# llsurreal919/Reduce-Complexity-for-intra-coding-of-VVC

Hardware: NVIDIA B200
Metric: all-intra 1080p10 CTUs/sec (exhaustive RMD sweep: intra pred + SAD/SATD + mode cost + candidate lists) (higher is better)
Workload: dtype int16 samples / int32 arithmetic / f64 costs

## Files before the change

### vvc_intra_b200/csrc/vvcb_core.cuh

```cuda
#pragma once
#include <stdint.h>
#include "../../include/vvc_intra_b200.h"

#if defined(__CUDACC__)
#define VHD __host__ __device__ __forceinline__
#else
#define VHD inline
#endif

namespace vvcb {

constexpr int kLineMax   = 140;
constexpr int kNumSets   = 4;
constexpr int kSlotLineWords = 54 * 32;
constexpr int kNumClasses = 6;
constexpr int kNumKinds   = 3;
constexpr int kNumBuckets = kNumClasses * kNumKinds;
#ifndef VVCB_ITEM_TASKS
#define VVCB_ITEM_TASKS 512
#endif
constexpr int kItemTasks = VVCB_ITEM_TASKS;

VHD int vmin(int a, int b) { return a < b ? a : b; }
VHD int vmax(int a, int b) { return a > b ? a : b; }
VHD int vabs(int a) { return a < 0 ? -a : a; }
VHD int vlog2(int v)
{
#if defined(__CUDA_ARCH__)
  return 31 - __clz(v);
#else
  return 31 - __builtin_clz((unsigned)v);
#endif
}
VHD int vsad(int a, int b, int c)
{
#if defined(__CUDA_ARCH__)
  return (int)__sad(a, b, (unsigned)c);
#else
  return c + (a < b ? b - a : a - b);
#endif
}

VHD uint32_t pack_u16x2(int lo, int hi) { return (uint32_t)lo | ((uint32_t)hi << 16); }
VHD uint32_t max_u16x2(uint32_t a, uint32_t b)
{
#if defined(__CUDA_ARCH__)
  return __vmaxu2(a, b);
#else
  const uint32_t al = a & 0xffffu, bl = b & 0xffffu, ah = a >> 16, bh = b >> 16;
  return (al > bl ? al : bl) | ((ah > bh ? ah : bh) << 16);
#endif
}
VHD int add_halves_u16x2(uint32_t w, int acc)
{
#if defined(__CUDA_ARCH__)
  return (int)__dp2a_lo(w, 0x00000101u, (unsigned)acc);
#else
  return acc + (int)(w & 0xffffu) + (int)(w >> 16);
#endif
}

struct ModeParam {
  int16_t  angle;
  uint16_t inv_angle;
  uint8_t  is_ver;
  uint8_t  ref_filter;
  uint8_t  interp;
  uint8_t  pdpc;
  int8_t   ang_scale;
  uint8_t  pad[3];
};

VHD int wide_angle(int w, int h, int mode)
{
  const int shiftTab[6] = { 0, 6, 10, 12, 14, 15 };
  if (mode > 1 && mode <= 66) {
    const int d = vabs(vlog2(w) - vlog2(h));
    if (w > h && mode < 2 + shiftTab[d]) mode += 65;
    else if (h > w && mode > 66 - shiftTab[d]) mode -= 65;
  }
  return mode;
}

VHD ModeParam make_mode_param(int w, int h, int mode, int mrl)
{
  const int angTab[32] = { 0, 1, 2, 3, 4, 6, 8, 10, 12, 14, 16, 18, 20, 23, 26, 29,
                           32, 35, 39, 45, 51, 57, 64, 73, 86, 102, 128, 171, 256, 341, 512, 1024 };
  const int invTab[32] = { 0, 16384, 8192, 5461, 4096, 2731, 2048, 1638, 1365, 1170, 1024, 910, 819, 712, 630, 565,
                           512, 468, 420, 364, 321, 287, 256, 224, 191, 161, 128, 96, 64, 48, 32, 16 };
  const int filtThr[8] = { 24, 24, 24, 14, 2, 0, 0, 0 };
  ModeParam p = {};
  const int predMode = wide_angle(w, h, mode);
  p.is_ver = predMode >= 34;
  p.pdpc   = mrl == 0;
  int absAng = 0;
  const int angMode = p.is_ver ? predMode - 50 : -(predMode - 18);
  if (mode > 1) {
    const int a = vabs(angMode);
    absAng      = angTab[a];
    p.inv_angle = (uint16_t)invTab[a];
    p.angle     = (int16_t)(angMode < 0 ? -absAng : absAng);
    if (angMode < 0) p.pdpc = 0;
    else if (angMode > 0) {
      const int side = p.is_ver ? h : w;
      const int sc   = vmin(2, vlog2(side) - (vlog2(3 * p.inv_angle - 2) - 8));
      p.ang_scale = (int8_t)sc;
      p.pdpc = p.pdpc && sc >= 0;
    }
  }
  if (mrl || mode == 1) return p;
  if (mode == 0) { p.ref_filter = w * h > 32; return p; }
// ... 53 lines not shown
  s.unitsX = w / s.S; s.unitsY = h / s.S;
  s.lanes = (s.tile == 1 || s.tile == 2) ? (w * h) / 32 : s.unitsX * s.unitsY;
  s.lgLanes  = vlog2(s.lanes);
  s.lgTilesX = s.S == 8 ? lw - 3 : (s.tile == 1 ? lw - 3 : lw - 2);
  return s;
}

struct WorkItem {
  uint32_t visit;
  uint16_t slot_begin;
  uint16_t slot_count;
};

struct LineGeom {
  int w, h, mrl, n;
  int lo[5], hi[5];
  int first;
};
constexpr int kNoInterval = 0x3fffffff;

VHD LineGeom make_line_geom(const vvcb_rmd_visit& v, int w, int h, int mrl)
{
  LineGeom g;
  g.w = w; g.h = h; g.mrl = mrl;
  const int C = 2 * h + 2 * mrl + 1;
  g.n = C + 2 * w;
  g.lo[0] = v.n_below_left  ? h - 4 * v.n_below_left : kNoInterval;  g.hi[0] = h;
  g.lo[1] = v.n_left        ? 2 * h - 4 * v.n_left   : kNoInterval;  g.hi[1] = 2 * h;
  g.lo[2] = v.avail_al      ? 2 * h                  : kNoInterval;  g.hi[2] = C;
  g.lo[3] = v.n_above       ? C                      : kNoInterval;  g.hi[3] = C + 4 * v.n_above;
  g.lo[4] = v.n_above_right ? C + w                  : kNoInterval;  g.hi[4] = C + w + 4 * v.n_above_right;
  g.first = -1;
#pragma unroll
  for (int k = 4; k >= 0; k--) if (g.lo[k] != kNoInterval) g.first = g.lo[k];
  return g;
}

VHD int line_source(const LineGeom& g, int i)
{
  int src = g.first;
#pragma unroll
  for (int k = 0; k < 5; k++)
    if (i >= g.lo[k]) src = i < g.hi[k] ? i : g.hi[k] - 1;
  return src;
}

VHD void line_pos(const LineGeom& g, int i, bool& isLeft, int& k, int& dx, int& dy)
{
  const int nLeft = 2 * g.h + g.mrl;
  if (i < nLeft) { isLeft = true;  k = nLeft - i;  dx = -1 - g.mrl; dy = -1 - g.mrl + k; }
  else           { isLeft = false; k = i - nLeft;  dx = -1 - g.mrl + k; dy = -1 - g.mrl; }
}

struct Rom {
  uint32_t filt[2][32];
  ModeParam mode[6][6][VVCB_NUM_LUMA_MODE];
  uint8_t angOrder[6][6][65];
  uint8_t mip4[18 * 16 * 4], mip8[10 * 16 * 8], mip16[6 * 64 * 7];
  uint8_t mipOff4[18], mipSh4[18], mipOff8[10], mipSh8[10], mipOff16[6], mipSh16[6];
};

template <int R, int C> VHD void wht_rows_rc(int (&d)[R][C])
{
#pragma unroll
  for (int y = 0; y < R; y++)
#pragma unroll
    for (int len = 1; len < C; len <<= 1)
#pragma unroll
      for (int i = 0; i < C; i += 2 * len)
#pragma unroll
        for (int x = i; x < i + len; x++) {
          const int a = d[y][x], b = d[y][x + len];
          d[y][x] = a + b; d[y][x + len] = a - b;
        }
}
template <int N> VHD void wht_rows(int (&d)[N][N]) { wht_rows_rc<N, N>(d); }

template <int R, int C> VHD void wht_cols_rc(int (&d)[R][C])
{
#pragma unroll
  for (int x = 0; x < C; x++)
#pragma unroll
    for (int len = 1; len < R; len <<= 1)
#pragma unroll
      for (int i = 0; i < R; i += 2 * len)
#pragma unroll
        for (int y = i; y < i + len; y++) {
          const int a = d[y][x], b = d[y + len][x];
          d[y][x] = a + b; d[y + len][x] = a - b;
        }
}

template <int N> VHD int wht_cols_abs_sum(int (&d)[N][N])
{
#pragma unroll
  for (int x = 0; x < N; x++)
#pragma unroll
    for (int len = 1; len < N / 2; len <<= 1)
#pragma unroll
      for (int i = 0; i < N; i += 2 * len)
#pragma unroll
        for (int y = i; y < i + len; y++) {
          const int a = d[y][x], b = d[y + len][x];
          d[y][x] = a + b; d[y + len][x] = a - b;
        }
  int s = 0;
#pragma unroll
  for (int x = 0; x < N; x++)
#pragma unroll
    for (int y = 0; y < N / 2; y++) s += vmax(vabs(d[y][x]), vabs(d[y + N / 2][x]));
  return 2 * s;
}
// ... 62 lines not shown
        }
      }
    } else {
      const int scale = p.ang_scale;
      const int lim = vmin(3 << scale, mw);
#pragma unroll
      for (int j = 0; j < C; j++) {
        const int c = c0 + j;
        if (c < lim) {
          const int wL  = 32 >> ((2 * c) >> scale);
          const int off = (256 + (c + 1) * (int)p.inv_angle) >> 9;
#pragma unroll
          for (int i = 0; i < R; i++) {
            const int l = side[r0 + i + off + 1];
            q[i][j] = q[i][j] + ((wL * (l - q[i][j]) + 32) >> 6);
          }
        }
      }
    }
  }
}

template <int R, int C> VHD void pred_planar_dc_unit(const int16_t* top, const int16_t* left, int kind, bool pdpc, int dc,
                                                     int lw, int lh, int x0, int y0, int (&b)[R][C])
{
  const int w = 1 << lw, h = 1 << lh;
  const int tr = top[w + 1], bl = left[h + 1];
  const int scale = (lw + lh - 2) >> 2;
#pragma unroll
  for (int i = 0; i < R; i++) {
    const int y = y0 + i;
    const int l = left[y + 1];
    const int wT = 32 >> vmin(31, (y << 1) >> scale);
#pragma unroll
    for (int j = 0; j < C; j++) {
      const int x = x0 + j;
      const int t = top[x + 1];
      int v;
      if (kind == 0) {
        const int hor = (l << lw) + (x + 1) * (tr - l);
        const int ver = (t << lh) + (y + 1) * (bl - t);
        v = ((hor << lh) + (ver << lw) + (1 << (lw + lh))) >> (1 + lw + lh);
      } else v = dc;
      if (pdpc) {
        const int wL = 32 >> vmin(31, (x << 1) >> scale);
        v = v + ((wL * (l - v) + wT * (t - v) + 32) >> 6);
      }
      b[i][j] = v;
    }
  }
}

struct MipGeom {
  int numModes, small, bsz, redW, redH, upH, upV, grid, cols;
  int lgRedW, lgUpH, lgUpV;
  int family;
};

VHD MipGeom make_mip_geom(int w, int h)
{
  MipGeom g;
  g.numModes = mip_num_modes(w, h);
  g.small = w <= 8 && h <= 8;
  g.bsz   = (w > 4 || h > 4) ? 4 : 2;
  g.redW  = g.small ? 4 : vmin(w, 8);
  g.redH  = g.small ? 4 : vmin(h, 8);
  g.upH   = w / g.redW; g.upV = h / g.redH;
  g.grid  = g.small ? 4 : 8;
  g.cols  = (w == 4 && h == 4) ? 4 : (g.small ? 8 : 7);
  g.lgRedW = vlog2(g.redW); g.lgUpH = vlog2(g.upH); g.lgUpV = vlog2(g.upV);
  g.family = (w == 4 && h == 4) ? 0 : (g.small ? 1 : 2);
  return g;
}

struct MipSlot {
  const uint8_t* mat;
  int shift, off, inOff;
  bool transpose;
  int in[8];
};

VHD MipSlot make_mip_slot(const Rom& rom, const MipGeom& g, const int16_t (*mipIn)[8], const int* mipAux, int mode)
{
  MipSlot m;
  m.transpose = mode > g.numModes / 2;
  const int widx = m.transpose ? mode - g.numModes / 2 : mode;
  int offs;
  if (g.family == 0)      { m.mat = rom.mip4 + widx * 64;   m.shift = rom.mipSh4[widx];  offs = rom.mipOff4[widx]; }
  else if (g.family == 1) { m.mat = rom.mip8 + widx * 128;  m.shift = rom.mipSh8[widx];  offs = rom.mipOff8[widx]; }
  else                    { m.mat = rom.mip16 + widx * 448; m.shift = rom.mipSh16[widx]; offs = rom.mipOff16[widx]; }
  const int t = m.transpose ? 1 : 0;
#pragma unroll
  for (int i = 0; i < 8; i++) m.in[i] = mipIn[t][i];
  m.inOff = mipAux[t];
  m.off = (1 << (m.shift - 1)) - offs * mipAux[2 + t];
  return m;
}

VHD int mip_reduced_sample(const MipSlot& m, const MipGeom& g, int w, int h, int maxv, int rx, int ry)
{
  bool lho = (w == 4 && h >= 16), lvo = (h == 4 && w >= 16);
  int xx = rx, yy = ry, iw = g.redW;
  if (m.transpose) { const bool t = lho; lho = lvo; lvo = t; xx = ry; yy = rx; iw = g.redH; }
  const int row = (lvo ? 2 * yy : yy) * (g.small ? iw : g.grid) + (lho ? 2 * xx : xx);
  const uint8_t* wgt = m.mat + row * g.cols;
  int acc = m.off;
  if (g.family == 0) {
#pragma unroll
    for (int i = 0; i < 4; i++) acc += m.in[i] * wgt[i];
  } else if (g.family == 1) {
#pragma unroll
    for (int i = 0; i < 8; i++) acc += m.in[i] * wgt[i];
  } else {
#pragma unroll
    for (int i = 1; i < 8; i++) acc += m.in[i] * wgt[i - 1];
  }
  return clip_bd((acc >> m.shift) + m.inOff, maxv);
}

VHD int trunc_bin_len(int symbol, int numSymbols)
{
  const int thresh = vlog2(numSymbols);
  const int b = numSymbols - (1 << thresh);
  return symbol < (1 << thresh) - b ? thresh : thresh + 1;
}

VHD uint64_t mode_bits(const vvcb_rates& r, const uint8_t* mpm, int w, int h, bool mrlAllowed, bool mipEnabled,
                       bool isMip, int mrl, int mode)
{
  const uint64_t EP = 1u << 15;
  uint64_t bits = 0;
  const int numMip = mip_num_modes(w, h);
  if (mipEnabled && numMip) bits += r.mip_flag[isMip ? 1 : 0];
  if (isMip) return bits + EP * (uint64_t)trunc_bin_len(mode, numMip);
  if (mrlAllowed) {
    bits += r.mrl_bin0[mrl != 0];
    if (mrl != 0) bits += r.mrl_bin1[mrl != 1];
  }
  if (mrl == 0 && vlog2(w) + vlog2(h) > 4) bits += r.isp_bin0_0;
  int idx = 6;
  for (int i = 5; i >= 0; i--) if (mpm[i] == mode) idx = i;
  if (mrl == 0) bits += r.mpm_flag[idx < 6];
  if (idx < 6) {
    if (mrl == 0) bits += r.planar_flag[idx > 0];
    if (idx > 0) bits += EP * (uint64_t)vmin(idx, 4);
  } else {
    int rem = mode;
    int below = 0;
    for (int i = 0; i < 6; i++) below += mpm[i] < mode;
    rem -= below;
    bits += EP * (uint64_t)trunc_bin_len(rem, 61);
  }
  return bits;
}

}
```

### vvc_intra_b200/csrc/vvcb_rmd.cuh

```cuda
#pragma once
#include "vvcb_core.cuh"

using namespace vvcb;

namespace {

#ifndef VVCB_EVAL_WARPS
#define VVCB_EVAL_WARPS 8
#endif
constexpr int kWarpsPerCta = VVCB_EVAL_WARPS;
constexpr int kThreads     = kWarpsPerCta * 32;
constexpr int KIND_ANG = 0, KIND_PDC = 1, KIND_MIP = 2;

template <int LMAX> struct VisitSmem {
  int16_t lines[kNumSets][2][LMAX];
  int16_t mipBnd[8];
  int16_t mipIn[2][8];
  int     mipAux[4];
  int     pad;
};
using WarpSmem = VisitSmem<kLineMax>;

#ifndef VVCB_PACK_VISITS
#define VVCB_PACK_VISITS 8
// ... 406 lines not shown
    const int16_t* row = org + r * stride;
#pragma unroll
    for (int c = 0; c < COLS; c += 4) {
      const uint2 v = *reinterpret_cast<const uint2*>(row + c);
      const int o0 = (int)(int16_t)(v.x & 0xffff), o1 = (int)(int16_t)(v.x >> 16);
      const int o2 = (int)(int16_t)(v.y & 0xffff), o3 = (int)(int16_t)(v.y >> 16);
      if (TRANSPOSED) {
        d[c + 0][r] = o0 - q[c + 0][r]; d[c + 1][r] = o1 - q[c + 1][r];
        d[c + 2][r] = o2 - q[c + 2][r]; d[c + 3][r] = o3 - q[c + 3][r];
        sad = vsad(o0, q[c + 0][r], sad); sad = vsad(o1, q[c + 1][r], sad);
        sad = vsad(o2, q[c + 2][r], sad); sad = vsad(o3, q[c + 3][r], sad);
      } else {
        d[r][c + 0] = o0 - q[r][c + 0]; d[r][c + 1] = o1 - q[r][c + 1];
        d[r][c + 2] = o2 - q[r][c + 2]; d[r][c + 3] = o3 - q[r][c + 3];
        sad = vsad(o0, q[r][c + 0], sad); sad = vsad(o1, q[r][c + 1], sad);
        sad = vsad(o2, q[r][c + 2], sad); sad = vsad(o3, q[r][c + 3], sad);
      }
    }
  }
}

template <int R, int C>
__device__ __forceinline__ void store_pred(int16_t* out, int w, int x0, int y0, bool transposed, const int (&q)[R][C])
{
#pragma unroll
  for (int i = 0; i < R; i++)
#pragma unroll
    for (int j = 0; j < C; j++) {
      if (transposed) out[(y0 + j) * w + x0 + i] = (int16_t)q[i][j];
      else            out[(y0 + i) * w + x0 + j] = (int16_t)q[i][j];
    }
}

template <int R, int C, class SM>
__device__ __forceinline__ void predict_angular(const SM& sm, const int16_t* projected, const SlotInfo& s, const Shape& sh,
                                                const uint32_t* filt, int bd, int x0, int y0, int rOff, int (&q)[R][C])
{
  const bool ver = s.p.is_ver;
  const int mw = ver ? sh.w : sh.h, mh = ver ? sh.h : sh.w;
  const int16_t* ml = s.p.angle < 0 ? projected + mh : sm.lines[s.set][ver ? 0 : 1];
  pred_angular_unit<R, C>(ml, sm.lines[s.set][ver ? 1 : 0], s.p, s.mrl, mw, mh, ver ? x0 : y0, (ver ? y0 : x0) + rOff, filt, (1 << bd) - 1, q);
}

__device__ __forceinline__ int mip_plane_offset(const MipGeom& mg, const Shape& sh)
{
  const bool identity = sh.h > sh.w ? mg.upH == 1 : mg.upV == 1;
  return identity ? 0 : mg.redW * mg.redH;
}

template <class SM>
__device__ void build_mip_planes(int16_t* red, int16_t* plane, const Rom& rom, const SM& sm, const MipGeom& mg, const Shape& sh,
                                 int bd, int mode, int gl, int gsize)
{
  const MipSlot ms = make_mip_slot(rom, mg, sm.mipIn, sm.mipAux, mode);
  const int nRed = mg.redW * mg.redH, maxv = (1 << bd) - 1;
  for (int i = gl; i < nRed; i += gsize)
    red[i] = (int16_t)mip_reduced_sample(ms, mg, sh.w, sh.h, maxv, i & (mg.redW - 1), i >> mg.lgRedW);
  __syncwarp();
  if (plane == red) return;
  const int16_t* top = sm.lines[0][0];
  const int16_t* left = sm.lines[0][1];
  if (sh.h > sh.w) {
    const int n = mg.redH << sh.lw;
    for (int i = gl; i < n; i += gsize) {
      const int ry = i >> sh.lw, x = i & (sh.w - 1);
      const int rx = x >> mg.lgUpH, k = (x & (mg.upH - 1)) + 1;
      const int row = mg.upV * (ry + 1) - 1;
      const int before = rx == 0 ? left[1 + row] : red[(ry << mg.lgRedW) + rx - 1];
      const int behind = red[(ry << mg.lgRedW) + rx];
      plane[i] = (int16_t)(((mg.upH - k) * before + k * behind + (mg.upH >> 1)) >> mg.lgUpH);
    }
  } else {
    const int n = sh.h << mg.lgRedW;
    for (int i = gl; i < n; i += gsize) {
      const int y = i >> mg.lgRedW, rx = i & (mg.redW - 1);
      const int ry = y >> mg.lgUpV, k = (y & (mg.upV - 1)) + 1;
      const int col = mg.upH * (rx + 1) - 1;
      const int before = ry == 0 ? top[1 + col] : red[((ry - 1) << mg.lgRedW) + rx];
      const int behind = red[(ry << mg.lgRedW) + rx];
      plane[i] = (int16_t)(((mg.upV - k) * before + k * behind + (mg.upV >> 1)) >> mg.lgUpV);
    }
  }
}

template <int R, int C, class SM>
__device__ __forceinline__ void predict_mip(const SM& sm, const int16_t* plane, const MipGeom& mg, const Shape& sh,
                                            int x0, int y0, int (&q)[R][C])
{
  const int16_t* top = sm.lines[0][0];
  const int16_t* left = sm.lines[0][1];
  if (sh.h > sh.w) {
#pragma unroll
    for (int i = 0; i < R; i++) {
      const int y = y0 + i;
      const int ry = y >> mg.lgUpV, k = (y & (mg.upV - 1)) + 1;
      const int16_t* rowB = plane + (ry << sh.lw) + x0;
#pragma unroll
      for (int j = 0; j < C; j++) {
        const int before = ry == 0 ? top[1 + x0 + j] : rowB[j - sh.w];
        q[i][j] = ((mg.upV - k) * before + k * rowB[j] + (mg.upV >> 1)) >> mg.lgUpV;
      }
    }
  } else {
#pragma unroll
    for (int i = 0; i < R; i++) {
      const int y = y0 + i;
      const int16_t* rowP = plane + (y << mg.lgRedW);
#pragma unroll
      for (int j = 0; j < C; j++) {
        const int x = x0 + j;
        const int rx = x >> mg.lgUpH, k = (x & (mg.upH - 1)) + 1;
        const int before = rx == 0 ? left[1 + y] : rowP[rx - 1];
        q[i][j] = ((mg.upH - k) * before + k * rowP[rx] + (mg.upH >> 1)) >> mg.lgUpH;
      }
    }
  }
}

#ifndef VVCB_EVAL_MIN_CTAS
#define VVCB_EVAL_MIN_CTAS 2
#endif
template <bool PACK> struct EvalCfg {
  static constexpr int kWarps   = PACK ? kWarpsPerCta / 2 : kWarpsPerCta;
  static constexpr int kThreads = kWarps * 32;
  static constexpr int kMinCtas = PACK ? 2 * VVCB_EVAL_MIN_CTAS : VVCB_EVAL_MIN_CTAS;
  static constexpr int kVisits  = PACK ? kPackVisits : 1;
  using Smem = VisitSmem<PACK ? kLineSmall : kLineMax>;
};

__host__ __device__ __forceinline__ int pack_shape_count(int tile) { return tile == 1 || tile == 2 ? 2 : 1; }
__host__ __device__ __forceinline__ int pack_shape(int tile, int i)
{
  return tile == 0 ? 0 : tile == 1 ? (i ? 4 : 1) : tile == 2 ? (i ? 5 : 2) : tile == 3 ? 3 : tile == 4 ? 6 : 7;
}

template <bool PACK> struct EvalShared {
  using Cfg = EvalCfg<PACK>;
  typename Cfg::Smem smem[Cfg::kWarps][Cfg::kVisits];
  int16_t sScratch[Cfg::kWarps][kSlotLineWords];
  vvcb_rmd_visit sVisit[Cfg::kWarps][Cfg::kVisits];
  int sSlots[Cfg::kWarps][Cfg::kVisits + 1];
  unsigned sIndex[Cfg::kWarps][Cfg::kVisits];
  uint32_t sFilt[64];
};

template <int TILE, int KIND, int MODE>
__device__ __forceinline__ void rmd_eval_body(const EvalParams& P, EvalShared<MODE == 1>& shm)
{
  constexpr bool PACK = MODE == 1, WITH_PRED = MODE == 2;
  using Cfg = EvalCfg<PACK>;
  using SM = typename Cfg::Smem;
  constexpr int S = TILE < 3 ? 4 : 8;
  constexpr int V = Cfg::kVisits;
  auto& smem = shm.smem;
  auto& sScratch = shm.sScratch;
  auto& sVisit = shm.sVisit;
  auto& sSlots = shm.sSlots;
  auto& sIndex = shm.sIndex;
  auto& sFilt = shm.sFilt;
  const int lane = threadIdx.x & 31, warp = threadIdx.x >> 5;
  if (threadIdx.x < 64) sFilt[threadIdx.x] = (&P.rom->filt[0][0])[threadIdx.x];
  __syncthreads();
  const Rom& rom = *P.rom;

#pragma unroll 1
  for (int ps = 0; ps < (PACK ? pack_shape_count(TILE) : 1); ps++) {
  const int BUCKET = PACK ? kNumBuckets + pack_shape(TILE, ps) * kNumKinds + KIND : TILE * kNumKinds + KIND;
  const unsigned nItems = P.plan->count[BUCKET];
  const WorkItem* items = P.items + P.plan->offset[BUCKET];

  for (;;) {
    unsigned it = 0;
    if (lane == 0) it = atomicAdd(&P.plan->cursor[BUCKET], (unsigned)V);
    it = __shfl_sync(0xffffffffu, it, 0);
    if (it >= nItems) break;
    const int nv = PACK ? (int)(nItems - it < (unsigned)V ? nItems - it : (unsigned)V) : 1;
    const WorkItem item = items[it];
    __syncwarp();
#pragma unroll 1
    for (int i = lane; i < nv * 20; i += 32) {
      const int j = i / 20, k = i - j * 20;
      reinterpret_cast<uint32_t*>(&sVisit[warp][j])[k] = reinterpret_cast<const uint32_t*>(P.visits + items[it + j].visit)[k];
    }
    if (lane < nv) sIndex[warp][lane] = items[it + lane].visit;
    __syncwarp();
    const Shape sh = make_shape(sVisit[warp][0].log2w, sVisit[warp][0].log2h);
    const MipGeom mg = make_mip_geom(sh.w, sh.h);
    int maxSlots = PACK ? 0 : (int)item.slot_count;
    if (PACK) {
      int c = lane < nv ? kind_slot_count(sVisit[warp][lane], KIND, P.ctu) : 0;
      if (lane < V) sSlots[warp][lane] = c;
      for (int o = V >> 1; o > 0; o >>= 1) c = vmax(c, __shfl_xor_sync(0xffffffffu, c, o));
      maxSlots = __shfl_sync(0xffffffffu, c, 0);
    }

#pragma unroll 1
    for (int j = 0; j < nv; j++) {
      const vvcb_rmd_visit& v = sVisit[warp][j];
      SM& sm = smem[warp][j];
      int nSets = 1;
      if (KIND != KIND_MIP) {
        const int lastSlot = kind_slot(rom, v, KIND, PACK ? kind_slot_count(v, KIND, P.ctu) - 1 : item.slot_begin + item.slot_count - 1);
        if (lastSlot >= VVCB_SLOT_MRL1) nSets = 3;
      }
      if (KIND == KIND_PDC) {
        if (nSets == 3) build_line_sets<3>(sm, v, sh, P.reco, P.stride, P.bd, lane);
        else            build_line_sets<1>(sm, v, sh, P.reco, P.stride, P.bd, lane);
      } else {
#pragma unroll 1
        for (int q = 0; q < nSets; q++) build_line_set(sm, q ? q + 1 : 0, q == 2 ? 3 : q, v, sh, P.reco, P.stride, P.bd, lane);
      }
    }
    __syncwarp();
#pragma unroll 1
    for (int j = 0; j < nv; j++) {
      if (KIND != KIND_MIP) build_filtered_set(smem[warp][j], sh, lane);
      else                  build_mip_inputs(smem[warp][j], sh, mg, P.bd, lane);
    }
    __syncwarp();

    const int lanes = sh.lanes;
    const int gsize = lanes > 32 ? 32 : lanes;
    const int lgG   = lanes > 32 ? 5 : sh.lgLanes;
    const int gidx  = lane >> lgG, gl = lane & (gsize - 1);
    int16_t* scratch = sScratch[warp] + gidx * ((kSlotLineWords / 32) << lgG);
    const int lgV = !PACK ? 0 : nv > 4 ? 3 : nv > 2 ? 2 : nv > 1 ? 1 : 0;
    const int nTasks = (maxSlots << lgV) * lanes;
    int accSad = 0, accSatd = 0;

    for (int base = 0; base < nTasks; base += 32) {
      const int task = base + lane;
      bool act = task < nTasks;
      int tk = act ? task : nTasks - 1;
      int vi = 0;
      if (PACK) {
        const int r = tk >> sh.lgLanes;
        vi = r & ((1 << lgV) - 1);
        int idx = r >> lgV;
        act = act && vi < nv && idx < sSlots[warp][vi];
        if (vi >= nv) vi = nv - 1;
        if (idx >= sSlots[warp][vi]) idx = sSlots[warp][vi] - 1;
        tk = (idx << sh.lgLanes) | (tk & (lanes - 1));
      }
      const vvcb_rmd_visit& v = sVisit[warp][vi];
      const SM& sm = smem[warp][vi];
      const unsigned vIdx = sIndex[warp][vi];
      const int16_t* org = P.orig + (size_t)v.y * P.stride + v.x;
      const int u = tk & (lanes - 1);
      const int slot = kind_slot(rom, v, KIND, (PACK ? 0 : item.slot_begin) + (tk >> sh.lgLanes));
      const SlotInfo s = make_slot_info(rom, v, sh, slot);

      __syncwarp();
      int dc = 0;
      if (KIND == KIND_ANG) {
        if (s.p.angle < 0) build_projected_line(scratch, sm, s, s.p.is_ver ? sh.w : sh.h, s.p.is_ver ? sh.h : sh.w, gl, gsize);
      } else if (KIND == KIND_MIP) {
        build_mip_planes(scratch, scratch + mip_plane_offset(mg, sh), rom, sm, mg, sh, P.bd, s.mode, gl, gsize);
      } else {
        int part = 0;
        if (s.kind == 1) {
          const int16_t* top = sm.lines[s.set][0] + s.mrl + 1;
          const int16_t* left = sm.lines[s.set][1] + s.mrl + 1;
          if (sh.w >= sh.h) for (int i = gl; i < sh.w; i += gsize) part += top[i];
          if (sh.w <= sh.h) for (int i = gl; i < sh.h; i += gsize) part += left[i];
        }
        for (int o = gsize >> 1; o > 0; o >>= 1) part += __shfl_xor_sync(0xffffffffu, part, o);
        const int denom = sh.w == sh.h ? 2 * sh.w : vmax(sh.w, sh.h);
        dc = (part + (denom >> 1)) >> vlog2(denom);
      }
      __syncwarp();

      int sad = 0, satd = 0;
      const bool transposed = KIND == KIND_ANG && !s.p.is_ver;
      if constexpr (S == 8) {
        const int ux = u & (sh.unitsX - 1), uy = u >> sh.lgTilesX;
        const int x0 = ux * 8, y0 = uy * 8;
        const int partnerMask = TILE == 4 ? 1 : sh.unitsX;
        const bool owner = TILE == 4 ? (ux & 1) == 0 : (uy & 1) == 0;
        uint32_t c0[4][4];
        int t = 0;
#pragma unroll 1
        for (int k = 0; k < 2; k++) {
          int q[4][8], d[4][8];
          const int hx = transposed ? x0 + 4 * k : x0, hy = transposed ? y0 : y0 + 4 * k;
          if (KIND == KIND_ANG)      predict_angular<4, 8>(sm, scratch, s, sh, sFilt, P.bd, x0, y0, 4 * k, q);
          else if (KIND == KIND_MIP) predict_mip<4, 8>(sm, scratch + mip_plane_offset(mg, sh), mg, sh, hx, hy, q);
          else pred_planar_dc_unit<4, 8>(sm.lines[s.set][0], sm.lines[s.set][1], s.kind, s.p.pdpc, dc, sh.lw, sh.lh, hx, hy, q);
          if (WITH_PRED && P.predOut && act) store_pred<4, 8>(P.predOut + (size_t)slot * sh.w * sh.h, sh.w, hx, hy, transposed, q);
          if (transposed) residual_unit<4, 8, true>(org + hy * P.stride + hx, P.stride, q, d, sad);
          else            residual_unit<4, 8, false>(org + hy * P.stride + hx, P.stride, q, d, sad);
          wht_rows_rc<4, 8>(d);
          wht_cols_rc<4, 8>(d);
          if (TILE != 3) {
#pragma unroll
            for (int i = 0; i < 4; i++)
#pragma unroll
              for (int j = 0; j < 8; j++) {
                const int other = __shfl_xor_sync(0xffffffffu, d[i][j], partnerMask);
                d[i][j] = owner ? d[i][j] + other : d[i][j] - other;
              }
          }
          if (k == 0) {
#pragma unroll
            for (int i = 0; i < 4; i++)
#pragma unroll
              for (int j = 0; j < 4; j++) c0[i][j] = pack_u16x2(vabs(d[i][2 * j]), vabs(d[i][2 * j + 1]));
          } else {
#pragma unroll
            for (int i = 0; i < 4; i++)
#pragma unroll
              for (int j = 0; j < 4; j++) t = add_halves_u16x2(max_u16x2(c0[i][j], pack_u16x2(vabs(d[i][2 * j]), vabs(d[i][2 * j + 1]))), t);
          }
        }
        if (TILE == 3) satd = (2 * t + 2) >> 2;
        else {
          t += __shfl_xor_sync(0xffffffffu, t, partnerMask);
          satd = owner ? satd_norm_rect(2 * t, true) : 0;
        }
      } else {
        const int tx = u & ((1 << sh.lgTilesX) - 1), ty = u >> sh.lgTilesX;
        uint32_t c0[4][2];
        int t = 0;
#pragma unroll
        for (int k = 0; k < (TILE == 0 ? 1 : 2); k++) {
          const int x0 = tx * (TILE == 1 ? 8 : 4) + (TILE == 1 ? 4 * k : 0);
          const int y0 = ty * (TILE == 2 ? 8 : 4) + (TILE == 2 ? 4 * k : 0);
          int q[4][4], d[4][4];
          if (KIND == KIND_ANG)      predict_angular<4, 4>(sm, scratch, s, sh, sFilt, P.bd, x0, y0, 0, q);
          else if (KIND == KIND_MIP) predict_mip<4, 4>(sm, scratch + mip_plane_offset(mg, sh), mg, sh, x0, y0, q);
          else pred_planar_dc_unit<4, 4>(sm.lines[s.set][0], sm.lines[s.set][1], s.kind, s.p.pdpc, dc, sh.lw, sh.lh, x0, y0, q);
          if (WITH_PRED && P.predOut && act) store_pred<4, 4>(P.predOut + (size_t)slot * sh.w * sh.h, sh.w, x0, y0, transposed, q);
          if (transposed) residual_unit<4, 4, true>(org + y0 * P.stride + x0, P.stride, q, d, sad);
          else            residual_unit<4, 4, false>(org + y0 * P.stride + x0, P.stride, q, d, sad);
          wht_rows<4>(d);
          if (TILE == 0) {
            satd = (wht_cols_abs_sum<4>(d) + 1) >> 1;
          } else {
            wht_cols<4>(d);
            if (k == 0) {
#pragma unroll
              for (int i = 0; i < 4; i++)
#pragma unroll
                for (int j = 0; j < 2; j++) c0[i][j] = pack_u16x2(vabs(d[i][2 * j]), vabs(d[i][2 * j + 1]));
            } else {
#pragma unroll
              for (int i = 0; i < 4; i++)
#pragma unroll
                for (int j = 0; j < 2; j++) t = add_halves_u16x2(max_u16x2(c0[i][j], pack_u16x2(vabs(d[i][2 * j]), vabs(d[i][2 * j + 1]))), t);
            }
          }
        }
        if (TILE != 0) satd = satd_norm_rect(2 * t, false);
      }
      if (!act) { sad = 0; satd = 0; }

      if (lanes <= 32) {
        for (int o = gsize >> 1; o > 0; o >>= 1) {
          sad  += __shfl_xor_sync(0xffffffffu, sad, o);
          satd += __shfl_xor_sync(0xffffffffu, satd, o);
        }
        if (act && gl == 0) {
          const size_t at = scratch_at(slot, vIdx, P.nVisits);
          if (P.satdSM) { P.sadSM[at] = (uint32_t)sad; P.satdSM[at] = (uint32_t)satd; }
          else P.sadSM[at] = (uint32_t)vmin(2 * sad, satd);
        }
      } else {
        accSad += sad; accSatd += satd;
        if (((base >> 5) & 1) == 1) {
          for (int o = 16; o > 0; o >>= 1) {
            accSad  += __shfl_xor_sync(0xffffffffu, accSad, o);
            accSatd += __shfl_xor_sync(0xffffffffu, accSatd, o);
          }
          if (lane == 0) {
            const size_t at = scratch_at(slot, vIdx, P.nVisits);
            if (P.satdSM) { P.sadSM[at] = (uint32_t)accSad; P.satdSM[at] = (uint32_t)accSatd; }
            else P.sadSM[at] = (uint32_t)vmin(2 * accSad, accSatd);
          }
          accSad = 0; accSatd = 0;
        }
      }
    }
  }
  }
}

template <int TILE, int KIND, int MODE>
__global__ void __launch_bounds__(EvalCfg<MODE == 1>::kThreads, EvalCfg<MODE == 1>::kMinCtas) rmd_eval_kernel(EvalParams P)
{
  __shared__ EvalShared<MODE == 1> shm;
  rmd_eval_body<TILE, KIND, MODE>(P, shm);
}

struct EvalAny {
  int n;
  int firstCta[19];
  unsigned char bucket[20];
};

template <int MODE>
__global__ void __launch_bounds__(EvalCfg<MODE == 1>::kThreads, EvalCfg<MODE == 1>::kMinCtas) rmd_eval_any_kernel(EvalParams P, EvalAny A)
{
  __shared__ EvalShared<MODE == 1> shm;
  int k = 0;
  while (k + 1 < A.n && (int)blockIdx.x >= A.firstCta[k + 1]) k++;
  switch (A.bucket[k]) {
    case 0:  rmd_eval_body<0, 0, MODE>(P, shm); break;  case 1:  rmd_eval_body<0, 1, MODE>(P, shm); break;  case 2:  rmd_eval_body<0, 2, MODE>(P, shm); break;
    case 3:  rmd_eval_body<1, 0, MODE>(P, shm); break;  case 4:  rmd_eval_body<1, 1, MODE>(P, shm); break;  case 5:  rmd_eval_body<1, 2, MODE>(P, shm); break;
    case 6:  rmd_eval_body<2, 0, MODE>(P, shm); break;  case 7:  rmd_eval_body<2, 1, MODE>(P, shm); break;  case 8:  rmd_eval_body<2, 2, MODE>(P, shm); break;
    case 9:  rmd_eval_body<3, 0, MODE>(P, shm); break;  case 10: rmd_eval_body<3, 1, MODE>(P, shm); break;  case 11: rmd_eval_body<3, 2, MODE>(P, shm); break;
    case 12: rmd_eval_body<4, 0, MODE>(P, shm); break;  case 13: rmd_eval_body<4, 1, MODE>(P, shm); break;  case 14: rmd_eval_body<4, 2, MODE>(P, shm); break;
    case 15: rmd_eval_body<5, 0, MODE>(P, shm); break;  case 16: rmd_eval_body<5, 1, MODE>(P, shm); break;  case 17: rmd_eval_body<5, 2, MODE>(P, shm); break;
  }
}

struct TuPredParams {
  const vvcb_rmd_visit* visits;
  const vvcb_tu_src*    src;
  const vvcb_tu_job*    jobs;
  int                   n;
  int16_t*              pred;
  int16_t*              resi;
  const int16_t*        orig;
  const int16_t*        reco;
  int                   stride, bd, ctu;
  const Rom*            rom;
};

constexpr int kTuPredWarps = 4;

__global__ void __launch_bounds__(kTuPredWarps * 32) tu_pred_kernel(TuPredParams P)
{
  __shared__ WarpSmem smem[kTuPredWarps];
  __shared__ int16_t sScratch[kTuPredWarps][kSlotLineWords];
  __shared__ uint32_t sFilt[64];
  const int lane = threadIdx.x & 31, warp = threadIdx.x >> 5;
  WarpSmem& sm = smem[warp];
  int16_t* const slotBuf = sScratch[warp];
  if (threadIdx.x < 64) sFilt[threadIdx.x] = (&P.rom->filt[0][0])[threadIdx.x];
  __syncthreads();
  const Rom& rom = *P.rom;
  for (int ji = blockIdx.x * kTuPredWarps + warp; ji < P.n; ji += gridDim.x * kTuPredWarps) {
    const vvcb_tu_src src = P.src[ji];
    const vvcb_rmd_visit v = P.visits[src.visit];
    const Shape sh = make_shape(v.log2w, v.log2h);
    const MipGeom mg = make_mip_geom(sh.w, sh.h);
    const int slot = src.slot;
    const SlotInfo s = make_slot_info(rom, v, sh, slot);
    const int16_t* org = P.orig + (size_t)v.y * P.stride + v.x;
    int16_t* predOut = P.pred + P.jobs[ji].offset;
    int16_t* resiOut = P.resi + P.jobs[ji].offset;
    __syncwarp();
    build_line_set(sm, 0, 0, v, sh, P.reco, P.stride, P.bd, lane);
    if (s.mrl) build_line_set(sm, s.set, s.mrl, v, sh, P.reco, P.stride, P.bd, lane);
    __syncwarp();
    if (s.kind != 3) build_filtered_set(sm, sh, lane);
    else             build_mip_inputs(sm, sh, mg, P.bd, lane);
    __syncwarp();
    int dc = 0;
    if (s.kind == 2) {
      if (s.p.angle < 0) build_projected_line(slotBuf, sm, s, s.p.is_ver ? sh.w : sh.h, s.p.is_ver ? sh.h : sh.w, lane, 32);
    } else if (s.kind == 3) {
      build_mip_planes(slotBuf, slotBuf + mip_plane_offset(mg, sh), rom, sm, mg, sh, P.bd, s.mode, lane, 32);
    } else if (s.kind == 1) {
      int part = 0;
// ... 493 lines not shown
```

### vvc_intra_b200/csrc/vvcb_romfill.h

```cpp
#pragma once
#include <string.h>
#include "vvcb_core.cuh"
#include "vvc_rom_tables.h"

namespace vvcb {
inline void fill_rom(Rom& r)
{
  memset(&r, 0, sizeof(r));
  for (int t = 0; t < 2; t++)
    for (int f = 0; f < 32; f++) {
      const int8_t* c = (t ? kIntraGaussFilter : kIntraCubicFilter) + 4 * f;
      r.filt[t][f] = (uint32_t)(uint8_t)c[0] | ((uint32_t)(uint8_t)c[1] << 8) | ((uint32_t)(uint8_t)c[2] << 16) | ((uint32_t)(uint8_t)c[3] << 24);
    }
  for (int lw = 2; lw <= 6; lw++)
    for (int lh = 2; lh <= 6; lh++)
      for (int m = 0; m < VVCB_NUM_LUMA_MODE; m++) r.mode[lw - 2][lh - 2][m] = make_mode_param(1 << lw, 1 << lh, m, 0);
  for (int lw = 2; lw <= 6; lw++)
    for (int lh = 2; lh <= 6; lh++) {
      int n = 0;
      for (int key = 0; key < 6; key++)
        for (int m = 2; m < VVCB_NUM_LUMA_MODE; m++) {
          const ModeParam& p = r.mode[lw - 2][lh - 2][m];
          const int cls = !p.pdpc ? 0 : (p.angle == 0 ? 2 : 1);
          if (p.is_ver * 3 + cls == key) r.angOrder[lw - 2][lh - 2][n++] = (uint8_t)m;
        }
    }
  memcpy(r.mip4, kMipMatrix4x4, sizeof(r.mip4));
  memcpy(r.mip8, kMipMatrix8x8, sizeof(r.mip8));
  memcpy(r.mip16, kMipMatrix16x16, sizeof(r.mip16));
  memcpy(r.mipOff4, kMipOffset4x4, 18); memcpy(r.mipSh4, kMipShift4x4, 18);
  memcpy(r.mipOff8, kMipOffset8x8, 10); memcpy(r.mipSh8, kMipShift8x8, 10);
  memcpy(r.mipOff16, kMipOffset16x16, 6); memcpy(r.mipSh16, kMipShift16x16, 6);
}

}

template <class T> inline void fill_tr_rom(T& r)
{
  memset(&r, 0, sizeof(r));
  memcpy(r.dct2, kDct2_4, 32); memcpy(r.dct2 + 16, kDct2_8, 128); memcpy(r.dct2 + 80, kDct2_16, 512);
  memcpy(r.dct2 + 336, kDct2_32, 2048); memcpy(r.dct2 + 1360, kDct2_64, 8192);
  memcpy(r.dct8, kDct8_4, 32); memcpy(r.dct8 + 16, kDct8_8, 128); memcpy(r.dct8 + 80, kDct8_16, 512); memcpy(r.dct8 + 336, kDct8_32, 2048);
  memcpy(r.dst7, kDst7_4, 32); memcpy(r.dst7 + 16, kDst7_8, 128); memcpy(r.dst7 + 80, kDst7_16, 512); memcpy(r.dst7 + 336, kDst7_32, 2048);
  for (int i = 0; i < 12; i++) { r.quantScales[i] = kQuantScales[i]; r.invQuantScales[i] = kInvQuantScales[i]; }
  memcpy(r.lfnst8, kLfnst8x8, sizeof(kLfnst8x8)); memcpy(r.lfnst4, kLfnst4x4, sizeof(kLfnst4x4)); memcpy(r.lfnstLut, kLfnstLut, 95);
  int n = 0;
  for (int d = 0; d <= 6; d++) for (int y = d < 3 ? d : 3; y >= 0 && d - y <= 3; y--) r.diag4[n++] = (uint8_t)((d - y) | (y << 2));
}

template <class T> inline void fill_dq_rom(T& r)
{
  memset(&r, 0, sizeof(r));
  static const int32_t riceBits[4][32] = {
    { 32768,  65536,  98304, 131072, 163840, 196608, 262144, 262144, 327680, 327680, 327680, 327680, 393216, 393216, 393216, 393216, 393216, 393216, 393216, 393216, 458752, 458752, 458752, 458752, 458752, 458752, 458752, 458752, 458752, 458752, 458752, 458752},
    { 65536,  65536,  98304,  98304, 131072, 131072, 163840, 163840, 196608, 196608, 229376, 229376, 294912, 294912, 294912, 294912, 360448, 360448, 360448, 360448, 360448, 360448, 360448, 360448, 425984, 425984, 425984, 425984, 425984, 425984, 425984, 425984},
    { 98304,  98304,  98304,  98304, 131072, 131072, 131072, 131072, 163840, 163840, 163840, 163840, 196608, 196608, 196608, 196608, 229376, 229376, 229376, 229376, 262144, 262144, 262144, 262144, 327680, 327680, 327680, 327680, 327680, 327680, 327680, 327680},
    {131072, 131072, 131072, 131072, 131072, 131072, 131072, 131072, 163840, 163840, 163840, 163840, 163840, 163840, 163840, 163840, 196608, 196608, 196608, 196608, 196608, 196608, 196608, 196608, 229376, 229376, 229376, 229376, 229376, 229376, 229376, 229376} };
  static const uint8_t ricePars[32] = { 0, 0, 0, 0, 0, 0, 0, 1, 1, 1, 1, 1, 1, 1, 2, 2, 2, 2, 2, 2, 2, 2, 2, 2, 2, 2, 2, 2, 3, 3, 3, 3 };
  static const uint8_t riceZero[3][32] = {
    {0, 0, 0, 0, 0, 1, 2, 2, 2, 2, 2, 2, 4, 4, 4, 4, 4, 4,  4,  4,  4,  4,  4,  8,  8,  8,  8,  8,  8,  8,  8,  8},
    {1, 1, 1, 1, 2, 3, 4, 4, 4, 6, 6, 6, 8, 8, 8, 8, 8, 8, 12, 12, 12, 12, 12, 12, 12, 12, 16, 16, 16, 16, 16, 16},
    {1, 1, 2, 2, 2, 3, 4, 4, 4, 6, 6, 6, 8, 8, 8, 8, 8, 8, 12, 12, 12, 12, 12, 12, 12, 16, 16, 16, 16, 16, 16, 16} };
  static const uint8_t groupIdx[32] = { 0,1,2,3,4,4,5,5,6,6,6,6,7,7,7,7,8,8,8,8,8,8,8,8,9,9,9,9,9,9,9,9 };
  memcpy(r.goRiceBits, riceBits, sizeof(riceBits)); memcpy(r.goRicePars, ricePars, 32); memcpy(r.goRiceZero, riceZero, 96);
  memcpy(r.groupIdx, groupIdx, 32);
  static const uint8_t tsRice[32] = { 0, 0, 0, 0, 0, 0, 0, 0, 0, 0, 0, 0, 1, 1, 1, 1, 1, 1, 1, 1, 1, 1, 1, 1, 1, 2, 2, 2, 2, 2, 2, 2 };
  memcpy(r.tsRicePars, tsRice, 32);
  for (int i = 0; i < 12; i++) { r.quantScales[i] = kQuantScales[i]; r.invQuantScales[i] = kInvQuantScales[i]; }

  auto diag = [](int bw, int bh, int* ox, int* oy) {
    int n = 0;
    for (int d = 0; d <= bw + bh - 2; d++)
      for (int y = (d < bh - 1 ? d : bh - 1); y >= 0 && d - y < bw; y--) { ox[n] = d - y; oy[n] = y; n++; }
    return n;
  };
  int ix[16], iy[16], inId[4][4];
  diag(4, 4, ix, iy);
  for (int i = 0; i < 16; i++) inId[iy[i]][ix[i]] = i;
  static const int dx[5] = { 1, 2, 1, 0, 0 }, dy[5] = { 0, 0, 1, 1, 2 };
  for (int i = 0; i < 16; i++) {
    int list[5], n = 0;
    for (int k = 0; k < 5; k++) { const int x = ix[i] + dx[k], y = iy[i] + dy[k]; if (x < 4 && y < 4) list[n++] = inId[y][x]; }
    for (int a = 1; a < n; a++) for (int b = a; b > 0 && list[b] < list[b - 1]; b--) { const int t = list[b]; list[b] = list[b - 1]; list[b - 1] = t; }
    r.nbIn[i][0] = (uint8_t)n;
    for (int k = 0; k < n; k++) r.nbIn[i][1 + k] = (uint8_t)list[k];
// ... 37 lines not shown
```

Measured before the change: 13380.

## Pack MIP weights as int8 words and compute MIP per lane with dp2a

The MIP matrices are repacked into 32-bit words of signed int8 weights plus a header word holding shift and offset. Reduced samples are now computed with dp2a dot products on packed int16 inputs. For small tiles (TILE<4, packed/pred modes) each lane computes MIP predictions directly, with interpolation carried across units, and the matrix family is staged in shared memory. This replaces the scratch-plane build and the scalar byte-weight loops. In exchange it adds shared memory per CTA and more register pressure, and the host aborts if any weight exceeds 127.

```diff
diff --git a/vvc_intra_b200/csrc/vvcb_core.cuh b/vvc_intra_b200/csrc/vvcb_core.cuh
--- a/vvc_intra_b200/csrc/vvcb_core.cuh
+++ b/vvc_intra_b200/csrc/vvcb_core.cuh
@@ -57,6 +57,23 @@
   return (int)__dp2a_lo(w, 0x00000101u, (unsigned)acc);
 #else
   return acc + (int)(w & 0xffffu) + (int)(w >> 16);
+#endif
+}
+
+VHD int dot2_s16_s8_lo(uint32_t a, uint32_t b, int c)
+{
+#if defined(__CUDA_ARCH__)
+  return __dp2a_lo((int)a, (int)b, c);
+#else
+  return c + (int)(int16_t)(a & 0xffffu) * (int)(int8_t)(b & 0xffu) + (int)(int16_t)(a >> 16) * (int)(int8_t)((b >> 8) & 0xffu);
+#endif
+}
+VHD int dot2_s16_s8_hi(uint32_t a, uint32_t b, int c)
+{
+#if defined(__CUDA_ARCH__)
+  return __dp2a_hi((int)a, (int)b, c);
+#else
+  return c + (int)(int16_t)(a & 0xffffu) * (int)(int8_t)((b >> 16) & 0xffu) + (int)(int16_t)(a >> 16) * (int)(int8_t)(b >> 24);
 #endif
 }
 
@@ -216,12 +233,16 @@
   else           { isLeft = false; k = i - nLeft;  dx = -1 - g.mrl + k; dy = -1 - g.mrl; }
 }
 
+VHD int mip_mode_words(int family) { return family == 0 ? 17 : (family == 1 ? 34 : 130); }
+VHD int mip_family_words(int family) { return family == 0 ? 18 * 17 : (family == 1 ? 10 * 34 : 6 * 130); }
+VHD int mip_family_base(int family) { return family == 0 ? 0 : (family == 1 ? 18 * 17 : 18 * 17 + 10 * 34); }
+constexpr int kMipRomWords = 18 * 17 + 10 * 34 + 6 * 130;
+
 struct Rom {
   uint32_t filt[2][32];
   ModeParam mode[6][6][VVCB_NUM_LUMA_MODE];
   uint8_t angOrder[6][6][65];
-  uint8_t mip4[18 * 16 * 4], mip8[10 * 16 * 8], mip16[6 * 64 * 7];
-  uint8_t mipOff4[18], mipSh4[18], mipOff8[10], mipSh8[10], mipOff16[6], mipSh16[6];
+  alignas(16) uint32_t mip[kMipRomWords];
 };
 
 template <int R, int C> VHD void wht_rows_rc(int (&d)[R][C])
@@ -390,7 +411,7 @@
 }
 
 struct MipGeom {
-  int numModes, small, bsz, redW, redH, upH, upV, grid, cols;
+  int numModes, small, bsz, redW, redH, upH, upV, grid;
   int lgRedW, lgUpH, lgUpV;
   int family;
 };
@@ -405,34 +426,50 @@
   g.redH  = g.small ? 4 : vmin(h, 8);
   g.upH   = w / g.redW; g.upV = h / g.redH;
   g.grid  = g.small ? 4 : 8;
-  g.cols  = (w == 4 && h == 4) ? 4 : (g.small ? 8 : 7);
   g.lgRedW = vlog2(g.redW); g.lgUpH = vlog2(g.upH); g.lgUpV = vlog2(g.upV);
   g.family = (w == 4 && h == 4) ? 0 : (g.small ? 1 : 2);
   return g;
 }
 
 struct MipSlot {
-  const uint8_t* mat;
+  const uint32_t* mat;
   int shift, off, inOff;
   bool transpose;
-  int in[8];
-};
-
-VHD MipSlot make_mip_slot(const Rom& rom, const MipGeom& g, const int16_t (*mipIn)[8], const int* mipAux, int mode)
+  uint32_t in[4];
+};
+
+VHD MipSlot make_mip_slot(const uint32_t* famRom, const MipGeom& g, const int16_t (*mipIn)[8], const int* mipAux, int mode)
 {
   MipSlot m;
   m.transpose = mode > g.numModes / 2;
   const int widx = m.transpose ? mode - g.numModes / 2 : mode;
-  int offs;
-  if (g.family == 0)      { m.mat = rom.mip4 + widx * 64;   m.shift = rom.mipSh4[widx];  offs = rom.mipOff4[widx]; }
-  else if (g.family == 1) { m.mat = rom.mip8 + widx * 128;  m.shift = rom.mipSh8[widx];  offs = rom.mipOff8[widx]; }
-  else                    { m.mat = rom.mip16 + widx * 448; m.shift = rom.mipSh16[widx]; offs = rom.mipOff16[widx]; }
+  m.mat = famRom + widx * mip_mode_words(g.family);
+  const uint32_t head = m.mat[g.family == 2 ? 128 : (g.family == 1 ? 32 : 16)];
+  m.shift = (int)(head & 0xffu);
   const int t = m.transpose ? 1 : 0;
-#pragma unroll
-  for (int i = 0; i < 8; i++) m.in[i] = mipIn[t][i];
+  const uint32_t* in2 = reinterpret_cast<const uint32_t*>(mipIn[t]);
+#pragma unroll
+  for (int i = 0; i < 4; i++) m.in[i] = in2[i];
   m.inOff = mipAux[t];
-  m.off = (1 << (m.shift - 1)) - offs * mipAux[2 + t];
+  m.off = (1 << (m.shift - 1)) - (int)(head >> 8) * mipAux[2 + t];
   return m;
+}
+
+template <bool WIDE> VHD int mip_row_sample(const MipSlot& m, int row, int maxv)
+{
+  int acc;
+  if (WIDE) {
+    const uint2 w = reinterpret_cast<const uint2*>(m.mat)[row];
+    acc = dot2_s16_s8_lo(m.in[0], w.x, m.off);
+    acc = dot2_s16_s8_hi(m.in[1], w.x, acc);
+    acc = dot2_s16_s8_lo(m.in[2], w.y, acc);
+    acc = dot2_s16_s8_hi(m.in[3], w.y, acc);
+  } else {
+    const uint32_t w = m.mat[row];
+    acc = dot2_s16_s8_lo(m.in[0], w, m.off);
+    acc = dot2_s16_s8_hi(m.in[1], w, acc);
+  }
+  return clip_bd((acc >> m.shift) + m.inOff, maxv);
 }
 
 VHD int mip_reduced_sample(const MipSlot& m, const MipGeom& g, int w, int h, int maxv, int rx, int ry)
@@ -441,19 +478,7 @@
   int xx = rx, yy = ry, iw = g.redW;
   if (m.transpose) { const bool t = lho; lho = lvo; lvo = t; xx = ry; yy = rx; iw = g.redH; }
   const int row = (lvo ? 2 * yy : yy) * (g.small ? iw : g.grid) + (lho ? 2 * xx : xx);
-  const uint8_t* wgt = m.mat + row * g.cols;
-  int acc = m.off;
-  if (g.family == 0) {
-#pragma unroll
-    for (int i = 0; i < 4; i++) acc += m.in[i] * wgt[i];
-  } else if (g.family == 1) {
-#pragma unroll
-    for (int i = 0; i < 8; i++) acc += m.in[i] * wgt[i];
-  } else {
-#pragma unroll
-    for (int i = 1; i < 8; i++) acc += m.in[i] * wgt[i - 1];
-  }
-  return clip_bd((acc >> m.shift) + m.inOff, maxv);
+  return g.family == 0 ? mip_row_sample<false>(m, row, maxv) : mip_row_sample<true>(m, row, maxv);
 }
 
 VHD int trunc_bin_len(int symbol, int numSymbols)
diff --git a/vvc_intra_b200/csrc/vvcb_rmd.cuh b/vvc_intra_b200/csrc/vvcb_rmd.cuh
--- a/vvc_intra_b200/csrc/vvcb_rmd.cuh
+++ b/vvc_intra_b200/csrc/vvcb_rmd.cuh
@@ -482,7 +482,7 @@
 __device__ void build_mip_planes(int16_t* red, int16_t* plane, const Rom& rom, const SM& sm, const MipGeom& mg, const Shape& sh,
                                  int bd, int mode, int gl, int gsize)
 {
-  const MipSlot ms = make_mip_slot(rom, mg, sm.mipIn, sm.mipAux, mode);
+  const MipSlot ms = make_mip_slot(rom.mip + mip_family_base(mg.family), mg, sm.mipIn, sm.mipAux, mode);
   const int nRed = mg.redW * mg.redH, maxv = (1 << bd) - 1;
   for (int i = gl; i < nRed; i += gsize)
     red[i] = (int16_t)mip_reduced_sample(ms, mg, sh.w, sh.h, maxv, i & (mg.redW - 1), i >> mg.lgRedW);
@@ -547,6 +547,55 @@
   }
 }
 
+template <int TILE, int R, int C, class SM>
+__device__ __forceinline__ void predict_mip_lane(const SM& sm, const MipSlot& ms, int k, int maxv, int (&carry)[4], int (&q)[R][C])
+{
+  const int16_t* top = sm.lines[0][0];
+  const int16_t* left = sm.lines[0][1];
+  const int stepY = ms.transpose ? 1 : 4, stepX = ms.transpose ? 4 : 1;
+  if constexpr (TILE == 0) {
+#pragma unroll
+    for (int i = 0; i < 4; i++)
+#pragma unroll
+      for (int j = 0; j < 4; j++) q[i][j] = mip_row_sample<false>(ms, i * stepY + j * stepX, maxv);
+  } else if constexpr (TILE == 1) {
+#pragma unroll
+    for (int i = 0; i < 4; i++) {
+      const int b  = k ? carry[i] : left[1 + i];
+      const int r0 = mip_row_sample<true>(ms, i * stepY + 2 * k * stepX, maxv);
+      const int r1 = mip_row_sample<true>(ms, i * stepY + (2 * k + 1) * stepX, maxv);
+      q[i][0] = (b + r0 + 1) >> 1; q[i][1] = r0; q[i][2] = (r0 + r1 + 1) >> 1; q[i][3] = r1;
+      carry[i] = r1;
+    }
+  } else {
+    int v[4][4];
+#pragma unroll
+    for (int rx = 0; rx < 4; rx++) {
+      const int b  = k ? carry[rx] : top[TILE == 3 ? 2 + 2 * rx : 1 + rx];
+      const int r0 = mip_row_sample<true>(ms, 2 * k * stepY + rx * stepX, maxv);
+      const int r1 = mip_row_sample<true>(ms, (2 * k + 1) * stepY + rx * stepX, maxv);
+      v[0][rx] = (b + r0 + 1) >> 1; v[1][rx] = r0; v[2][rx] = (r0 + r1 + 1) >> 1; v[3][rx] = r1;
+      carry[rx] = r1;
+    }
+    if constexpr (TILE == 2) {
+#pragma unroll
+      for (int i = 0; i < 4; i++)
+#pragma unroll
+        for (int j = 0; j < 4; j++) q[i][j] = v[i][j];
+    } else {
+#pragma unroll
+      for (int i = 0; i < 4; i++) {
+        const int l = left[1 + 4 * k + i];
+#pragma unroll
+        for (int rx = 0; rx < 4; rx++) {
+          q[i][2 * rx]     = ((rx ? v[i][rx - 1] : l) + v[i][rx] + 1) >> 1;
+          q[i][2 * rx + 1] = v[i][rx];
+        }
+      }
+    }
+  }
+}
+
 #ifndef VVCB_EVAL_MIN_CTAS
 #define VVCB_EVAL_MIN_CTAS 2
 #endif
@@ -574,14 +623,20 @@
   uint32_t sFilt[64];
 };
 
+template <int TILE, int KIND, int MODE> constexpr bool kLaneMip = KIND == KIND_MIP && TILE < 4 && MODE != 0;
+constexpr int kMipLaneWords = 10 * 34;
+
 template <int TILE, int KIND, int MODE>
-__device__ __forceinline__ void rmd_eval_body(const EvalParams& P, EvalShared<MODE == 1>& shm)
+__device__ __forceinline__ void rmd_eval_body(const EvalParams& P, EvalShared<MODE == 1>& shm, uint32_t* sMip)
 {
   constexpr bool PACK = MODE == 1, WITH_PRED = MODE == 2;
   using Cfg = EvalCfg<PACK>;
   using SM = typename Cfg::Smem;
   constexpr int S = TILE < 3 ? 4 : 8;
   constexpr int V = Cfg::kVisits;
+  constexpr bool LANE_MIP = kLaneMip<TILE, KIND, MODE>;
+  constexpr bool ONLY_LANE_MIP = LANE_MIP && PACK && (TILE == 0 || TILE == 3);
+  constexpr int MIP_FAMILY = TILE == 0 ? 0 : 1;
   auto& smem = shm.smem;
   auto& sScratch = shm.sScratch;
   auto& sVisit = shm.sVisit;
@@ -590,6 +645,8 @@
   auto& sFilt = shm.sFilt;
   const int lane = threadIdx.x & 31, warp = threadIdx.x >> 5;
   if (threadIdx.x < 64) sFilt[threadIdx.x] = (&P.rom->filt[0][0])[threadIdx.x];
+  if (LANE_MIP)
+    for (int i = threadIdx.x; i < mip_family_words(MIP_FAMILY); i += Cfg::kThreads) sMip[i] = P.rom->mip[mip_family_base(MIP_FAMILY) + i];
   __syncthreads();
   const Rom& rom = *P.rom;
 
@@ -682,10 +739,11 @@
 
       __syncwarp();
       int dc = 0;
+      const bool laneMip = ONLY_LANE_MIP || (LANE_MIP && lanes == 1);
       if (KIND == KIND_ANG) {
         if (s.p.angle < 0) build_projected_line(scratch, sm, s, s.p.is_ver ? sh.w : sh.h, s.p.is_ver ? sh.h : sh.w, gl, gsize);
       } else if (KIND == KIND_MIP) {
-        build_mip_planes(scratch, scratch + mip_plane_offset(mg, sh), rom, sm, mg, sh, P.bd, s.mode, gl, gsize);
+        if (!laneMip) build_mip_planes(scratch, scratch + mip_plane_offset(mg, sh), rom, sm, mg, sh, P.bd, s.mode, gl, gsize);
       } else {
         int part = 0;
         if (s.kind == 1) {
@@ -702,6 +760,9 @@
 
       int sad = 0, satd = 0;
       const bool transposed = KIND == KIND_ANG && !s.p.is_ver;
+      MipSlot ms = {};
+      int mipCarry[4] = {};
+      if (laneMip) ms = make_mip_slot(sMip, mg, sm.mipIn, sm.mipAux, s.mode);
       if constexpr (S == 8) {
         const int ux = u & (sh.unitsX - 1), uy = u >> sh.lgTilesX;
         const int x0 = ux * 8, y0 = uy * 8;
@@ -714,6 +775,7 @@
           int q[4][8], d[4][8];
           const int hx = transposed ? x0 + 4 * k : x0, hy = transposed ? y0 : y0 + 4 * k;
           if (KIND == KIND_ANG)      predict_angular<4, 8>(sm, scratch, s, sh, sFilt, P.bd, x0, y0, 4 * k, q);
+          else if (KIND == KIND_MIP && laneMip) predict_mip_lane<TILE, 4, 8>(sm, ms, k, (1 << P.bd) - 1, mipCarry, q);
           else if (KIND == KIND_MIP) predict_mip<4, 8>(sm, scratch + mip_plane_offset(mg, sh), mg, sh, hx, hy, q);
           else pred_planar_dc_unit<4, 8>(sm.lines[s.set][0], sm.lines[s.set][1], s.kind, s.p.pdpc, dc, sh.lw, sh.lh, hx, hy, q);
           if (WITH_PRED && P.predOut && act) store_pred<4, 8>(P.predOut + (size_t)slot * sh.w * sh.h, sh.w, hx, hy, transposed, q);
@@ -757,6 +819,7 @@
           const int y0 = ty * (TILE == 2 ? 8 : 4) + (TILE == 2 ? 4 * k : 0);
           int q[4][4], d[4][4];
           if (KIND == KIND_ANG)      predict_angular<4, 4>(sm, scratch, s, sh, sFilt, P.bd, x0, y0, 0, q);
+          else if (KIND == KIND_MIP && laneMip) predict_mip_lane<TILE, 4, 4>(sm, ms, k, (1 << P.bd) - 1, mipCarry, q);
           else if (KIND == KIND_MIP) predict_mip<4, 4>(sm, scratch + mip_plane_offset(mg, sh), mg, sh, x0, y0, q);
           else pred_planar_dc_unit<4, 4>(sm.lines[s.set][0], sm.lines[s.set][1], s.kind, s.p.pdpc, dc, sh.lw, sh.lh, x0, y0, q);
           if (WITH_PRED && P.predOut && act) store_pred<4, 4>(P.predOut + (size_t)slot * sh.w * sh.h, sh.w, x0, y0, transposed, q);
@@ -818,7 +881,10 @@
 __global__ void __launch_bounds__(EvalCfg<MODE == 1>::kThreads, EvalCfg<MODE == 1>::kMinCtas) rmd_eval_kernel(EvalParams P)
 {
   __shared__ EvalShared<MODE == 1> shm;
-  rmd_eval_body<TILE, KIND, MODE>(P, shm);
+  if constexpr (kLaneMip<TILE, KIND, MODE>) {
+    alignas(16) __shared__ uint32_t sMip[kMipLaneWords];
+    rmd_eval_body<TILE, KIND, MODE>(P, shm, sMip);
+  } else rmd_eval_body<TILE, KIND, MODE>(P, shm, nullptr);
 }
 
 struct EvalAny {
@@ -831,15 +897,16 @@
 __global__ void __launch_bounds__(EvalCfg<MODE == 1>::kThreads, EvalCfg<MODE == 1>::kMinCtas) rmd_eval_any_kernel(EvalParams P, EvalAny A)
 {
   __shared__ EvalShared<MODE == 1> shm;
+  alignas(16) __shared__ uint32_t sMip[MODE == 0 ? 1 : kMipLaneWords];
   int k = 0;
   while (k + 1 < A.n && (int)blockIdx.x >= A.firstCta[k + 1]) k++;
   switch (A.bucket[k]) {
-    case 0:  rmd_eval_body<0, 0, MODE>(P, shm); break;  case 1:  rmd_eval_body<0, 1, MODE>(P, shm); break;  case 2:  rmd_eval_body<0, 2, MODE>(P, shm); break;
-    case 3:  rmd_eval_body<1, 0, MODE>(P, shm); break;  case 4:  rmd_eval_body<1, 1, MODE>(P, shm); break;  case 5:  rmd_eval_body<1, 2, MODE>(P, shm); break;
-    case 6:  rmd_eval_body<2, 0, MODE>(P, shm); break;  case 7:  rmd_eval_body<2, 1, MODE>(P, shm); break;  case 8:  rmd_eval_body<2, 2, MODE>(P, shm); break;
-    case 9:  rmd_eval_body<3, 0, MODE>(P, shm); break;  case 10: rmd_eval_body<3, 1, MODE>(P, shm); break;  case 11: rmd_eval_body<3, 2, MODE>(P, shm); break;
-    case 12: rmd_eval_body<4, 0, MODE>(P, shm); break;  case 13: rmd_eval_body<4, 1, MODE>(P, shm); break;  case 14: rmd_eval_body<4, 2, MODE>(P, shm); break;
-    case 15: rmd_eval_body<5, 0, MODE>(P, shm); break;  case 16: rmd_eval_body<5, 1, MODE>(P, shm); break;  case 17: rmd_eval_body<5, 2, MODE>(P, shm); break;
+    case 0:  rmd_eval_body<0, 0, MODE>(P, shm, sMip); break;  case 1:  rmd_eval_body<0, 1, MODE>(P, shm, sMip); break;  case 2:  rmd_eval_body<0, 2, MODE>(P, shm, sMip); break;
+    case 3:  rmd_eval_body<1, 0, MODE>(P, shm, sMip); break;  case 4:  rmd_eval_body<1, 1, MODE>(P, shm, sMip); break;  case 5:  rmd_eval_body<1, 2, MODE>(P, shm, sMip); break;
+    case 6:  rmd_eval_body<2, 0, MODE>(P, shm, sMip); break;  case 7:  rmd_eval_body<2, 1, MODE>(P, shm, sMip); break;  case 8:  rmd_eval_body<2, 2, MODE>(P, shm, sMip); break;
+    case 9:  rmd_eval_body<3, 0, MODE>(P, shm, sMip); break;  case 10: rmd_eval_body<3, 1, MODE>(P, shm, sMip); break;  case 11: rmd_eval_body<3, 2, MODE>(P, shm, sMip); break;
+    case 12: rmd_eval_body<4, 0, MODE>(P, shm, sMip); break;  case 13: rmd_eval_body<4, 1, MODE>(P, shm, sMip); break;  case 14: rmd_eval_body<4, 2, MODE>(P, shm, sMip); break;
+    case 15: rmd_eval_body<5, 0, MODE>(P, shm, sMip); break;  case 16: rmd_eval_body<5, 1, MODE>(P, shm, sMip); break;  case 17: rmd_eval_body<5, 2, MODE>(P, shm, sMip); break;
   }
 }
 
diff --git a/vvc_intra_b200/csrc/vvcb_romfill.h b/vvc_intra_b200/csrc/vvcb_romfill.h
--- a/vvc_intra_b200/csrc/vvcb_romfill.h
+++ b/vvc_intra_b200/csrc/vvcb_romfill.h
@@ -1,4 +1,5 @@
 #pragma once
+#include <stdlib.h>
 #include <string.h>
 #include "vvcb_core.cuh"
 #include "vvc_rom_tables.h"
@@ -25,12 +26,23 @@
           if (p.is_ver * 3 + cls == key) r.angOrder[lw - 2][lh - 2][n++] = (uint8_t)m;
         }
     }
-  memcpy(r.mip4, kMipMatrix4x4, sizeof(r.mip4));
-  memcpy(r.mip8, kMipMatrix8x8, sizeof(r.mip8));
-  memcpy(r.mip16, kMipMatrix16x16, sizeof(r.mip16));
-  memcpy(r.mipOff4, kMipOffset4x4, 18); memcpy(r.mipSh4, kMipShift4x4, 18);
-  memcpy(r.mipOff8, kMipOffset8x8, 10); memcpy(r.mipSh8, kMipShift8x8, 10);
-  memcpy(r.mipOff16, kMipOffset16x16, 6); memcpy(r.mipSh16, kMipShift16x16, 6);
+  static const uint8_t* const mat[3] = { kMipMatrix4x4, kMipMatrix8x8, kMipMatrix16x16 };
+  static const uint8_t* const off[3] = { kMipOffset4x4, kMipOffset8x8, kMipOffset16x16 };
+  static const uint8_t* const sh[3] = { kMipShift4x4, kMipShift8x8, kMipShift16x16 };
+  static const int modes[3] = { 18, 10, 6 }, rows[3] = { 16, 16, 64 }, cols[3] = { 4, 8, 7 };
+  for (int f = 0; f < 3; f++)
+    for (int m = 0; m < modes[f]; m++) {
+      uint32_t* dst = r.mip + mip_family_base(f) + m * mip_mode_words(f);
+      const int rowWords = f ? 2 : 1;
+      for (int y = 0; y < rows[f]; y++)
+        for (int c = 0; c < cols[f]; c++) {
+          const uint8_t wgt = mat[f][(m * rows[f] + y) * cols[f] + c];
+          if (wgt > 127) abort();
+          const int k = c + (f == 2 ? 1 : 0);
+          dst[y * rowWords + (k >> 2)] |= (uint32_t)wgt << (8 * (k & 3));
+        }
+      dst[rows[f] * rowWords] = (uint32_t)sh[f][m] | ((uint32_t)off[f][m] << 8);
+    }
 }
 
 }
```

Measured after the change: 14120, median of 6. +5.5%, better.
